# ChenKaiXuSan/Skiing_Analysis_PyTorch

Hardware: AMD Instinct MI355X
Metric: 3D-pose frames/sec, 8-view 518px clips (higher is better)
Workload: dtype f16

## Files before the change

skiing_analysis_pytorch_amd/csrc/common.h:

```cpp
#pragma once
#include <hip/hip_runtime.h>
#include <stdint.h>
#include <stdio.h>
#include <atomic>
#include <string>

#include "../../include/skimi.h"

namespace skimi {

void set_error(const char* fmt, ...);

#define SKIMI_CHECK_ARG(cond, ...)            \
    do {                                      \
        if (!(cond)) {                        \
            ::skimi::set_error(__VA_ARGS__);  \
            return SKIMI_ERR_ARG;             \
        }                                     \
    } while (0)

#define SKIMI_HIP(call)                                                                  \
    do {                                                                                 \
        hipError_t e_ = (call);                                                          \
        if (e_ != hipSuccess) {                                                          \
            ::skimi::set_error("%s failed: %s (%s:%d)", #call, hipGetErrorString(e_),    \
                               __FILE__, __LINE__);                                      \
            return SKIMI_ERR_HIP;                                                        \
        }                                                                                \
    } while (0)

#define SKIMI_LAUNCH_CHECK()                                                             \
    do {                                                                                 \
        hipError_t e_ = hipGetLastError();                                               \
        if (e_ != hipSuccess) {                                                          \
            ::skimi::set_error("kernel launch failed: %s (%s:%d)", hipGetErrorString(e_),\
                               __FILE__, __LINE__);                                      \
            return SKIMI_ERR_HIP;                                                        \
        }                                                                                \
    } while (0)

enum ProfKind { PROF_NONE = 0, PROF_ATTN_BF16 = 1, PROF_GEMM = 2 };
bool prof_armed(int kind, long size_key);
void prof_before(hipStream_t st);
void prof_after(hipStream_t st, double flops, double bytes);

int lds_opt_in(std::atomic<unsigned>& done, const void* kernel, int bytes, const char* what);
#define SKIMI_LDS_OPT_IN(KERNEL, BYTES, WHAT)                                                            \
    do {                                                                                                 \
        static std::atomic<unsigned> done_{0};                                                           \
        const int rc_ = ::skimi::lds_opt_in(done_, reinterpret_cast<const void*>(KERNEL), (int)(BYTES), WHAT); \
        if (rc_ != SKIMI_OK) return rc_;                                                                 \
    } while (0)

static inline int64_t cdiv(int64_t a, int64_t b) { return (a + b - 1) / b; }
static inline size_t align_up(size_t a, size_t b) { return (a + b - 1) / b * b; }

typedef __attribute__((ext_vector_type(8))) short bf16x8;
typedef __attribute__((ext_vector_type(4))) short bf16x4;
typedef __attribute__((ext_vector_type(16))) float f32x16;
typedef __attribute__((ext_vector_type(4))) float f32x4;

#ifdef __HIPCC__
__device__ __forceinline__ unsigned short f2bf(float x) {
    __bf16 b = (__bf16)x;
    return __builtin_bit_cast(unsigned short, b);
}
__device__ __forceinline__ float bf2f(unsigned short b) {
    return __builtin_bit_cast(float, ((unsigned int)b) << 16);
}
__device__ __forceinline__ unsigned short f2h(float x) {
    _Float16 h = (_Float16)x;
    return __builtin_bit_cast(unsigned short, h);
}
__device__ __forceinline__ float h2f(unsigned short b) { return (float)__builtin_bit_cast(_Float16, b); }
__device__ __forceinline__ unsigned short f2x16(float x, bool f16) {
    const unsigned short a = f2h(x), b = f2bf(x);
    return f16 ? a : b;
}
__device__ __forceinline__ float x16tof(unsigned short b, bool f16) {
    const float a = h2f(b), c = bf2f(b);
    return f16 ? a : c;
}
typedef __attribute__((ext_vector_type(8))) _Float16 f16x8;
template <bool F16>
__device__ __forceinline__ f32x16 mfma_32x32x16(bf16x8 a, bf16x8 b, f32x16 c) {
    if constexpr (F16)
        return __builtin_amdgcn_mfma_f32_32x32x16_f16(__builtin_bit_cast(f16x8, a), __builtin_bit_cast(f16x8, b), c, 0, 0, 0);
    else
        return __builtin_amdgcn_mfma_f32_32x32x16_bf16(a, b, c, 0, 0, 0);
}
__device__ __forceinline__ unsigned mx_scale_byte(float amax) {
    if (!(amax > 0.f)) return 0u;
    const float t = amax * (1.0f / 448.0f);
    const unsigned u = __float_as_uint(t);
    const int e = (int)((u >> 23) & 0xFF) - 127 + ((u & 0x7FFFFF) ? 1 : 0);
    return (unsigned)min(max(e + 127, 1), 254);
}
__device__ __forceinline__ float mx_inv_scale(unsigned sb) { return sb ? __uint_as_float((unsigned)(254 - (int)sb) << 23) : 0.f; }
__device__ __forceinline__ int mx_pack4(float a, float b, float c, float d, float inv) {
    int w = 0;
    w = __builtin_amdgcn_cvt_pk_fp8_f32(a * inv, b * inv, w, false);
    w = __builtin_amdgcn_cvt_pk_fp8_f32(c * inv, d * inv, w, true);
    return w;
}
__device__ __forceinline__ float max8(float v) {
    int x = __float_as_int(v);
    v = fmaxf(v, __int_as_float(__builtin_amdgcn_update_dpp(x, x, 0xB1, 0xF, 0xF, true)));
    x = __float_as_int(v);
    v = fmaxf(v, __int_as_float(__builtin_amdgcn_update_dpp(x, x, 0x4E, 0xF, 0xF, true)));
    x = __float_as_int(v);
    v = fmaxf(v, __int_as_float(__builtin_amdgcn_update_dpp(x, x, 0x141, 0xF, 0xF, true)));
    return v;
}
__device__ __forceinline__ float wave_sum(float v) {
#pragma unroll
    for (int o = 32; o > 0; o >>= 1) v += __shfl_xor(v, o, 64);
    return v;
}
__device__ __forceinline__ float wave_max(float v) {
#pragma unroll
    for (int o = 32; o > 0; o >>= 1) v = fmaxf(v, __shfl_xor(v, o, 64));
    return v;
}
#endif

}
```

skiing_analysis_pytorch_amd/csrc/gemm256.hip:

```cpp
#include <stdlib.h>

#include "common.h"
#include "gemm_epilogue.h"

namespace skimi {

typedef __attribute__((address_space(3))) void lds_void;
typedef __attribute__((address_space(1))) const void gbl_void;

__device__ __forceinline__ void tile_coords256(const GemmArgs& p, int& tm, int& tn) {
    const int nblk = p.ntm * p.ntn;
    const int bid = blockIdx.x;
    const int xcd = bid & 7;
    const int q = nblk >> 3, r = nblk & 7;
    const int id = (xcd < r ? xcd * (q + 1) : r * (q + 1) + (xcd - r) * q) + (bid >> 3);
    constexpr int GM = 8;
    const int per_group = GM * p.ntn;
    const int group = id / per_group, within = id - group * per_group;
    const int rows = min(GM, p.ntm - group * GM);
    tn = within / rows;
    tm = group * GM + within - tn * rows;
}

template <bool H16>
__device__ __forceinline__ bf16x4 pack4_16(float y0, float y1, float y2, float y3) {
    bf16x4 hb;
    if constexpr (H16) {
        hb[0] = (short)f2h(y0); hb[1] = (short)f2h(y1); hb[2] = (short)f2h(y2); hb[3] = (short)f2h(y3);
    } else {
        hb[0] = (short)f2bf(y0); hb[1] = (short)f2bf(y1); hb[2] = (short)f2bf(y2); hb[3] = (short)f2bf(y3);
    }
    return hb;
}

template <int MT, int EPI, int PF = 2, bool H16 = false>
__device__ __forceinline__ void epilogue256(const GemmArgs& p, f32x16 (&acc)[MT][2], char* smem, int wave, int lane,
                                            int wr, int wc, int m0, int n0) {
    const int l31 = lane & 31, lh = lane >> 5;
    float* stg = reinterpret_cast<float*>(smem) + wave * (32 * 64);
    const int n = n0 + wc * 64 + 4 * (lane & 15);
    if (p.dbg & 8) {
        if (acc[0][0][0] == 123.456f) ((float*)p.out)[0] = acc[MT - 1][1][15];
        return;
    }
    const bool interior = (m0 + 64 * MT <= p.M) && (n0 + 256 <= p.N) && !(p.dbg & 4);
    float4 bs = make_float4(0, 0, 0, 0), gm = make_float4(1, 1, 1, 1);
    if (EPI != 0 && n < p.N) {
        if (p.bias) bs = *reinterpret_cast<const float4*>(p.bias + n);
        if (EPI == 2) gm = *reinterpret_cast<const float4*>(p.gamma + n);
    }
#define SKIMI_ACC_TO_SLAB(i)                                                                                   \
    do {                                                                                                        \
        _Pragma("unroll") for (int j = 0; j < 2; ++j) _Pragma("unroll") for (int r = 0; r < 16; ++r)            \
            stg[((r & 3) + 8 * (r >> 2) + 4 * lh) * 64 + j * 32 + l31] = acc[i][j][r];                         \
        __builtin_amdgcn_fence(__ATOMIC_RELEASE, "wavefront");                                                  \
        __builtin_amdgcn_s_waitcnt(0xC07F);                                                     \
    } while (0)

    if (EPI == 2 && interior) {
        const int mrow0 = m0 + wr * (32 * MT) + (lane >> 4);
        float4 r[PF][8];
#pragma unroll
        for (int i = 0; i < PF && i < MT; ++i)
#pragma unroll
            for (int it = 0; it < 8; ++it)
                r[i][it] = *reinterpret_cast<const float4*>((const float*)p.resid + (long)(mrow0 + i * 32 + it * 4) * p.ldr + n);
#pragma unroll
        for (int i = 0; i < MT; ++i) {
            SKIMI_ACC_TO_SLAB(i);
            const int mrow = mrow0 + i * 32;
            float4 v[8];
#pragma unroll
            for (int it = 0; it < 8; ++it)
                v[it] = *reinterpret_cast<const float4*>(&stg[(it * 4 + (lane >> 4)) * 64 + 4 * (lane & 15)]);
#pragma unroll
            for (int it = 0; it < 8; ++it) {
                const float4 rr = r[i % PF][it];
                f32x4 ov = {rr.x + gm.x * (v[it].x + bs.x), rr.y + gm.y * (v[it].y + bs.y),
                            rr.z + gm.z * (v[it].z + bs.z), rr.w + gm.w * (v[it].w + bs.w)};
                *reinterpret_cast<f32x4*>((float*)p.out + (long)(mrow + it * 4) * p.ldo + n) = ov;
            }
            if (i + PF < MT) {
#pragma unroll
                for (int it = 0; it < 8; ++it)
                    r[i % PF][it] =
                        *reinterpret_cast<const float4*>((const float*)p.resid + (long)(mrow + PF * 32 + it * 4) * p.ldr + n);
            }
            __builtin_amdgcn_s_waitcnt(0xC07F);
        }
        return;
    }
    if (EPI != 0 && interior) {
        const bool mx = EPI == 3 && p.out_dtype == SKIMI_FP8MX;
#pragma unroll
        for (int i = 0; i < MT; ++i) {
            SKIMI_ACC_TO_SLAB(i);
            const int mrow = m0 + wr * (32 * MT) + i * 32 + (lane >> 4);
            float4 v[8];
#pragma unroll
            for (int it = 0; it < 8; ++it)
                v[it] = *reinterpret_cast<const float4*>(&stg[(it * 4 + (lane >> 4)) * 64 + 4 * (lane & 15)]);
            unsigned sb_mine = 0;
#pragma unroll
            for (int it = 0; it < 8; ++it) {
                float y0 = v[it].x + bs.x, y1 = v[it].y + bs.y, y2 = v[it].z + bs.z, y3 = v[it].w + bs.w;
                if (EPI == 3) {
                    const f32x2_t g0 = gelu_erf2(f32x2_t{y0, y1}), g1 = gelu_erf2(f32x2_t{y2, y3});
                    y0 = g0.x; y1 = g0.y; y2 = g1.x; y3 = g1.y;
                }
                if (mx) {
                    const unsigned sb = mx_scale_byte(max8(fmaxf(fmaxf(fabsf(y0), fabsf(y1)), fmaxf(fabsf(y2), fabsf(y3)))));
                    const long row = mrow + it * 4;
                    *reinterpret_cast<int*>((unsigned char*)p.out + row * p.ldo + n) = mx_pack4(y0, y1, y2, y3, mx_inv_scale(sb));
                    sb_mine = (lane & 7) == it ? sb : sb_mine;
                    if (it == 7) p.out_scales[(long)(mrow + (lane & 7) * 4) * (p.N >> 5) + (n >> 5)] = (unsigned char)sb_mine;
                    continue;
                }
                *reinterpret_cast<bf16x4*>((unsigned short*)p.out + (long)(mrow + it * 4) * p.ldo + n) = pack4_16<H16>(y0, y1, y2, y3);
            }
            __builtin_amdgcn_s_waitcnt(0xC07F);
        }
        return;
    }
#pragma unroll
    for (int i = 0; i < MT; ++i) {
        SKIMI_ACC_TO_SLAB(i);
        const int mrow = m0 + wr * (32 * MT) + i * 32 + (lane >> 4);
        if (EPI != 0) {
#pragma unroll 1
            for (int it = 0; it < 8; ++it) {
                const int m = mrow + it * 4;
                if (m >= p.M || n >= p.N || (p.dbg & 4)) continue;
                const float4 v = *reinterpret_cast<const float4*>(&stg[(it * 4 + (lane >> 4)) * 64 + 4 * (lane & 15)]);
                float y0 = v.x + bs.x, y1 = v.y + bs.y, y2 = v.z + bs.z, y3 = v.w + bs.w;
                if (EPI == 2) {
                    const float4 r = *reinterpret_cast<const float4*>((const float*)p.resid + (long)m * p.ldr + n);
                    f32x4 ov = {r.x + gm.x * y0, r.y + gm.y * y1, r.z + gm.z * y2, r.w + gm.w * y3};
// ... 59 lines not shown
    const unsigned short* w_src[4];
#pragma unroll
    for (int j = 0; j < MT; ++j) {
        const int row = 8 * (MT * wave + j) + (lane >> 3);
        const int c = (lane & 7) ^ ((row >> 1) & 7);
        a_src[j] = A + (long)min(m0 + row, p.M - 1) * p.lda + c * 8;
    }
#pragma unroll
    for (int j = 0; j < 4; ++j) {
        const int row = 8 * (4 * wave + j) + (lane >> 3);
        const int c = (lane & 7) ^ ((row >> 1) & 7);
        w_src[j] = W + (long)min(n0 + row, p.N - 1) * p.ldw + c * 8;
    }
    auto stage = [&](int buf, int kt) {
        char* ab = smem + buf * BUF + (MT * wave) * 8 * RB;
        char* wb = smem + buf * BUF + A_TILE + (4 * wave) * 8 * RB;
#pragma unroll
        for (int j = 0; j < MT; ++j)
            __builtin_amdgcn_global_load_lds((gbl_void*)(a_src[j] + kt * BK), (lds_void*)(ab + j * 8 * RB), 16, 0, 0);
#pragma unroll
        for (int j = 0; j < 4; ++j)
            __builtin_amdgcn_global_load_lds((gbl_void*)(w_src[j] + kt * BK), (lds_void*)(wb + j * 8 * RB), 16, 0, 0);
    };

    f32x16 acc[MT][2];
#pragma unroll
    for (int i = 0; i < MT; ++i)
#pragma unroll
        for (int j = 0; j < 2; ++j)
#pragma unroll
            for (int r = 0; r < 16; ++r) acc[i][j][r] = 0.f;

    stage(0, 0);
    __syncthreads();
    for (int kt = 0; kt < nkt; ++kt) {
        const int cur = kt & 1;
        if (kt + 1 < nkt && !(p.dbg & 1)) stage(cur ^ 1, kt + 1);
        const char* ab = smem + cur * BUF;
        const char* wb = ab + A_TILE;
        bf16x8 af[2][MT], wf[2][2];
        auto load_frags = [&](int s, int set) {
#pragma unroll
            for (int i = 0; i < MT; ++i) {
                const int row = wr * (32 * MT) + i * 32 + l31;
                af[set][i] = *reinterpret_cast<const bf16x8*>(ab + row * RB + (((2 * s + lh) ^ ((row >> 1) & 7)) << 4));
            }
#pragma unroll
            for (int j = 0; j < 2; ++j) {
                const int row = wc * 64 + j * 32 + l31;
                wf[set][j] = *reinterpret_cast<const bf16x8*>(wb + row * RB + (((2 * s + lh) ^ ((row >> 1) & 7)) << 4));
            }
        };
        if (!(p.dbg & 2)) {
        load_frags(0, 0);
        __builtin_amdgcn_sched_barrier(0);
#pragma unroll
        for (int s = 0; s < 4; ++s) {
            if (s + 1 < 4) load_frags(s + 1, (s + 1) & 1);
            __builtin_amdgcn_sched_barrier(0);
            __builtin_amdgcn_s_setprio(1);
#pragma unroll
            for (int i = 0; i < MT; ++i)
#pragma unroll
                for (int j = 0; j < 2; ++j)
                    acc[i][j] = mfma_32x32x16<F16>(af[s & 1][i], wf[s & 1][j], acc[i][j]);
            __builtin_amdgcn_s_setprio(0);
            __builtin_amdgcn_sched_barrier(0);
        }
        }
        __syncthreads();
    }

    epilogue256<MT, EPI, 2, F16 && EPI == 3>(p, acc, smem, wave, lane, wr, wc, m0, n0);
}

#define SKIMI_BAR()                           \
    do {                                      \
        __builtin_amdgcn_sched_barrier(0);    \
        __builtin_amdgcn_s_barrier();         \
        __builtin_amdgcn_sched_barrier(0);    \
    } while (0)
#define SKIMI_VMCNT(N) __builtin_amdgcn_s_waitcnt(0x0F70 | ((N) & 15) | (((N) >> 4) << 14))

template <int EPI, int DEEP, bool F16 = false>
__global__ __launch_bounds__(512, 2) void gemm256pp_kernel(const GemmArgs p) {
    constexpr int MT = 4, BM = 256, BN = 256, BK = 64;
    constexpr int RB = 128;
    constexpr int A_TILE = BM * RB, W_TILE = BN * RB, BUF = A_TILE + W_TILE;
    extern __shared__ __attribute__((aligned(16))) char smem[];

    const int tid = threadIdx.x, lane = tid & 63;
    const int wave = __builtin_amdgcn_readfirstlane(tid >> 6);
    const int wr = wave >> 2, wc = wave & 3;
    const int l31 = lane & 31, lh = lane >> 5;

    int tm, tn;
    tile_coords256(p, tm, tn);
    const int m0 = tm * BM, n0 = tn * BN;
    const int nkt = p.K / BK;

    const unsigned short* A = (const unsigned short*)p.A;
    const unsigned short* W = (const unsigned short*)p.W;
    const unsigned short* a_src[2][2];
    const unsigned short* w_src[2][2];
    int a_row0[2][2], w_row0[2][2];
#pragma unroll
    for (int h = 0; h < 2; ++h)
#pragma unroll
        for (int j = 0; j < 2; ++j) {
            const int g = 2 * wave + j;
            a_row0[h][j] = (g >> 3) * 128 + 64 * h + 8 * (g & 7);
            w_row0[h][j] = (g >> 2) * 64 + 32 * h + 8 * (g & 3);
            int row = a_row0[h][j] + (lane >> 3);
            int c = (lane & 7) ^ ((row >> 1) & 7);
            a_src[h][j] = A + (long)min(((p.dbg & 64) ? 0 : m0) + row, p.M - 1) * p.lda + c * 8;
            row = w_row0[h][j] + (lane >> 3);
            c = (lane & 7) ^ ((row >> 1) & 7);
            w_src[h][j] = W + (long)min(((p.dbg & 64) ? 0 : n0) + row, p.N - 1) * p.ldw + c * 8;
        }
    const bool no_dma = p.dbg & 1, no_mfma = p.dbg & 2, no_rd = p.dbg & 32;
    auto issue_a = [&](int h, int kt) {
        if (no_dma) return;
        char* base = smem + (kt & 1) * BUF;
#pragma unroll
        for (int j = 0; j < 2; ++j)
            __builtin_amdgcn_global_load_lds((gbl_void*)(a_src[h][j] + kt * BK), (lds_void*)(base + a_row0[h][j] * RB), 16,
                                             0, 0);
    };
    auto issue_w = [&](int h, int kt) {
        if (no_dma) return;
        char* base = smem + (kt & 1) * BUF + A_TILE;
#pragma unroll
        for (int j = 0; j < 2; ++j)
            __builtin_amdgcn_global_load_lds((gbl_void*)(w_src[h][j] + kt * BK), (lds_void*)(base + w_row0[h][j] * RB), 16,
                                             0, 0);
    };

    f32x16 acc[MT][2];
#pragma unroll
    for (int i = 0; i < MT; ++i)
#pragma unroll
        for (int j = 0; j < 2; ++j)
#pragma unroll
            for (int r = 0; r < 16; ++r) acc[i][j][r] = 0.f;

    issue_a(0, 0); issue_w(0, 0); issue_w(1, 0); issue_a(1, 0);
    if (nkt > 1) {
        issue_a(0, 1);
        if (DEEP) issue_w(0, 1);
        issue_w(1, 1);
        if (DEEP) SKIMI_VMCNT(6); else SKIMI_VMCNT(4);
    } else {
        SKIMI_VMCNT(0);
    }
    SKIMI_BAR();
    if (wr == 1) SKIMI_BAR();

    bf16x8 af[2][4], wf[2][4];
    if (no_rd) {
#pragma unroll
        for (int i = 0; i < 2; ++i)
#pragma unroll
            for (int s = 0; s < 4; ++s) af[i][s] = wf[i][s] = bf16x8{0, 0, 0, 0, 0, 0, 0, 0};
    }
    for (int kt = 0; kt < nkt; ++kt) {
        const char* ab = smem + (kt & 1) * BUF;
        const char* wb = ab + A_TILE;
        auto read_a = [&](int ih) {
            if (no_rd) return;
#pragma unroll
            for (int i = 0; i < 2; ++i)
#pragma unroll
                for (int s = 0; s < 4; ++s) {
                    const int row = wr * 128 + (2 * ih + i) * 32 + l31;
                    af[i][s] = *reinterpret_cast<const bf16x8*>(ab + row * RB + (((2 * s + lh) ^ ((row >> 1) & 7)) << 4));
                }
        };
        auto read_w = [&](int jh) {
            if (no_rd) return;
#pragma unroll
            for (int s = 0; s < 4; ++s) {
                const int row = wc * 64 + jh * 32 + l31;
                wf[jh][s] = *reinterpret_cast<const bf16x8*>(wb + row * RB + (((2 * s + lh) ^ ((row >> 1) & 7)) << 4));
            }
        };
#define SKIMI_QUADRANT(IH, JH)                                                                                  \
    do {                                                                                                         \
        SKIMI_BAR();                                                                                             \
        __builtin_amdgcn_s_setprio(1);                                                                           \
        if (!no_mfma) _Pragma("unroll") for (int s = 0; s < 4; ++s) {                                                          \
            acc[2 * IH][JH] = mfma_32x32x16<F16>(af[0][s], wf[JH][s], acc[2 * IH][JH]);                           \
            acc[2 * IH + 1][JH] = mfma_32x32x16<F16>(af[1][s], wf[JH][s], acc[2 * IH + 1][JH]);                   \
        }                                                                                                        \
        __builtin_amdgcn_s_setprio(0);                                                                           \
        SKIMI_BAR();                                                                                             \
    } while (0)

        read_w(0);
        read_a(0);
        if (kt + 1 < nkt) issue_a(1, kt + 1);
        SKIMI_QUADRANT(0, 0);
        read_w(1);
        if (!DEEP && kt + 1 < nkt) issue_w(0, kt + 1);
        SKIMI_QUADRANT(0, 1);
        read_a(1);
        if (kt + 2 < nkt) {
            issue_a(0, kt + 2);
            if (DEEP) issue_w(0, kt + 2);
        }
        SKIMI_QUADRANT(1, 1);
        if (kt + 2 < nkt) {
            issue_w(1, kt + 2);
            if (DEEP) SKIMI_VMCNT(6); else SKIMI_VMCNT(4);
        } else {
            SKIMI_VMCNT(0);
        }
        SKIMI_QUADRANT(1, 0);
#undef SKIMI_QUADRANT
    }
    if (wr == 0) SKIMI_BAR();

    epilogue256<MT, EPI, 2, F16 && EPI == 3>(p, acc, smem, wave, lane, wr, wc, m0, n0);
}


template <int EPI, bool F16 = false>
__global__ __launch_bounds__(256, 1) void gemm256w4_kernel(const GemmArgs p) {
    constexpr int RB = 128, BK = 64, PIECE = 128 * RB, NSLOT = 10;
    extern __shared__ __attribute__((aligned(16))) char smem[];

    const int tid = threadIdx.x, lane = tid & 63;
    const int wave = __builtin_amdgcn_readfirstlane(tid >> 6);
    const int wr = wave >> 1, wc = wave & 1;
    const int l31 = lane & 31, lh = lane >> 5;

    int tm, tn;
    tile_coords256(p, tm, tn);
    const int m0 = tm * 256, n0 = tn * 256;
    const int nkt = p.K / BK;
    const unsigned short* src[4][4];
#pragma unroll
    for (int q = 0; q < 4; ++q)
#pragma unroll
        for (int j = 0; j < 4; ++j) {
            const int row = (4 * wave + j) * 8 + (lane >> 3);
            const int c = (lane & 7) ^ ((row >> 1) & 7);
            src[q][j] = q < 2 ? (const unsigned short*)p.A + (long)min(m0 + 128 * q + row, p.M - 1) * p.lda + c * 8
                              : (const unsigned short*)p.W + (long)min(n0 + 128 * (q - 2) + row, p.N - 1) * p.ldw + c * 8;
        }
    auto issue = [&](int q, int kt, int slot) {
        char* base = smem + slot * PIECE + (4 * wave) * 8 * RB;
#pragma unroll
        for (int j = 0; j < 4; ++j)
            __builtin_amdgcn_global_load_lds((gbl_void*)(src[q][j] + kt * BK), (lds_void*)(base + j * 8 * RB), 16, 0, 0);
    };

    const int t = lh ^ ((l31 >> 1) & 7);
    const int lane_off = l31 * RB;
    bf16x8 fa0[4], fb0[4], fa1[4], fb1[4];
    auto read = [&](int sb, int s, bf16x8 (&fa)[4], bf16x8 (&fb)[4]) {
        int sa = sb + wr, sw = sb + 2 + wc;
        sa = sa >= NSLOT ? sa - NSLOT : sa;
        sw = sw >= NSLOT ? sw - NSLOT : sw;
        const char* pa = smem + sa * PIECE + lane_off + (((2 * s) ^ t) << 4);
        const char* pw = smem + sw * PIECE + lane_off + (((2 * s) ^ t) << 4);
#pragma unroll
        for (int i = 0; i < 4; ++i) fa[i] = *reinterpret_cast<const bf16x8*>(pa + i * 32 * RB);
#pragma unroll
        for (int i = 0; i < 4; ++i) fb[i] = *reinterpret_cast<const bf16x8*>(pw + i * 32 * RB);
    };

    f32x16 acc[2][4][2];
#pragma unroll
    for (int h = 0; h < 2; ++h)
#pragma unroll
        for (int i = 0; i < 4; ++i)
#pragma unroll
            for (int j = 0; j < 2; ++j)
#pragma unroll
                for (int r = 0; r < 16; ++r) acc[h][i][j][r] = 0.f;
#define SKIMI_W4_MFMA(FA, FB)                                                                                   \
    _Pragma("unroll") for (int j = 0; j < 4; ++j) _Pragma("unroll") for (int i = 0; i < 4; ++i)                 \
        acc[j >> 1][i][j & 1] = mfma_32x32x16<F16>(FA[i], FB[j], acc[j >> 1][i][j & 1])

#pragma unroll
    for (int q = 0; q < 4; ++q) issue(q, 0, q);
    if (nkt > 1) {
#pragma unroll
        for (int q = 0; q < 4; ++q) issue(q, 1, 4 + q);
        SKIMI_VMCNT(16);
    } else {
        SKIMI_VMCNT(0);
    }
    SKIMI_BAR();
    int sb = 0;
    read(sb, 0, fa0, fb0);
#define SKIMI_W4_HEAD()                       \
    do {                                      \
        __builtin_amdgcn_s_waitcnt(0xC07F);   \
        __builtin_amdgcn_sched_barrier(0);    \
    } while (0)
#define SKIMI_W4_TAIL(NDMA)                                                        \
    do {                                                                           \
        _Pragma("unroll") for (int g = 0; g < 4; ++g) {                            \
            __builtin_amdgcn_sched_group_barrier(0x008, 1, 0);                     \
            __builtin_amdgcn_sched_group_barrier(0x100, 2, 0);                     \
        }                                                                          \
        _Pragma("unroll") for (int g = 0; g < NDMA; ++g) {                         \
            __builtin_amdgcn_sched_group_barrier(0x008, 1, 0);                     \
            __builtin_amdgcn_sched_group_barrier(0x010, 1, 0);                     \
        }                                                                          \
        __builtin_amdgcn_sched_group_barrier(0x008, 12 - NDMA, 0);                 \
        __builtin_amdgcn_sched_barrier(0);                                         \
    } while (0)
#define SKIMI_W4_KTILE(N1, N2)                                                      \
    do {                                                                            \
        int s8 = sb + 8, s9 = sb + 9, s1 = sb + 1, nsb = sb + 4;                    \
        s8 = s8 >= NSLOT ? s8 - NSLOT : s8;                                         \
        s9 = s9 >= NSLOT ? s9 - NSLOT : s9;                                         \
        s1 = s1 >= NSLOT ? s1 - NSLOT : s1;                                         \
        nsb = nsb >= NSLOT ? nsb - NSLOT : nsb;                                     \
                                                                      \
        SKIMI_W4_HEAD();                                                            \
        read(sb, 1, fa1, fb1);                                                      \
        SKIMI_W4_MFMA(fa0, fb0);                                                    \
        SKIMI_W4_TAIL(0);                                                           \
                                                                      \
        SKIMI_W4_HEAD();                                                            \
        read(sb, 2, fa0, fb0);                                                      \
        if (N2) issue(0, kt + 2, s8);                                               \
        SKIMI_W4_MFMA(fa1, fb1);                                                    \
        SKIMI_W4_TAIL((N2 ? 4 : 0));                                                \
                                                                      \
        SKIMI_W4_HEAD();                                                            \
        read(sb, 3, fa1, fb1);                                                      \
        if (N2) issue(1, kt + 2, s9);                                               \
        SKIMI_W4_MFMA(fa0, fb0);                                                    \
        SKIMI_W4_TAIL((N2 ? 4 : 0));                                                \
                                                                      \
        SKIMI_W4_HEAD();                                                            \
        if (N1) {                                                                   \
            if (N2) SKIMI_VMCNT(8); else SKIMI_VMCNT(0);                            \
            SKIMI_BAR();                                                            \
            read(nsb, 0, fa0, fb0);                                                 \
            if (N2) {                                                               \
                issue(2, kt + 2, sb);                                               \
                issue(3, kt + 2, s1);                                               \
            }                                                                       \
        }                                                                           \
        SKIMI_W4_MFMA(fa1, fb1);                                                    \
        if (N1) SKIMI_W4_TAIL((N2 ? 8 : 0)); else __builtin_amdgcn_sched_barrier(0); \
        sb = nsb;                                                                   \
    } while (0)
    int kt = 0;
    for (; kt + 2 < nkt; ++kt) SKIMI_W4_KTILE(true, true);
    if (kt + 1 < nkt) {
        SKIMI_W4_KTILE(true, false);
        ++kt;
    }
    SKIMI_W4_KTILE(false, false);
#undef SKIMI_W4_KTILE
#undef SKIMI_W4_HEAD
#undef SKIMI_W4_TAIL
#undef SKIMI_W4_MFMA
    __builtin_amdgcn_s_waitcnt(0xC07F);
    SKIMI_BAR();

    epilogue256<4, EPI, 4, F16 && EPI == 3>(p, acc[0], smem, wave, lane, wr, 2 * wc, m0, n0);
    epilogue256<4, EPI, 4, F16 && EPI == 3>(p, acc[1], smem, wave, lane, wr, 2 * wc + 1, m0, n0);
}


typedef __attribute__((ext_vector_type(8))) int i32x8_t;
typedef __attribute__((ext_vector_type(4))) int i32x4_t;

template <int EPI>
__global__ __launch_bounds__(256, 1) void gemm256w4_fp8_kernel(const GemmArgs p) {
    constexpr int RB = 128, BK = 128, PIECE = 128 * RB, NSLOT = 10;
    extern __shared__ __attribute__((aligned(16))) char smem[];

    const int tid = threadIdx.x, lane = tid & 63;
    const int wave = __builtin_amdgcn_readfirstlane(tid >> 6);
    const int wr = wave >> 1, wc = wave & 1;
    const int l31 = lane & 31, lh = lane >> 5;

    int tm, tn;
    tile_coords256(p, tm, tn);
    const int m0 = tm * 256, n0 = tn * 256;
    const int nkt = p.K / BK;
    const unsigned char* src[4][4];
#pragma unroll
    for (int q = 0; q < 4; ++q)
#pragma unroll
        for (int j = 0; j < 4; ++j) {
            const int row = (4 * wave + j) * 8 + (lane >> 3);
            const int c = (lane & 7) ^ ((row >> 1) & 7);
            src[q][j] = q < 2 ? (const unsigned char*)p.A + (long)min(m0 + 128 * q + row, p.M - 1) * p.lda + c * 16
                              : (const unsigned char*)p.W + (long)min(n0 + 128 * (q - 2) + row, p.N - 1) * p.ldw + c * 16;
        }
    auto issue = [&](int q, int kt, int slot) {
        char* base = smem + slot * PIECE + (4 * wave) * 8 * RB;
#pragma unroll
        for (int j = 0; j < 4; ++j)
            __builtin_amdgcn_global_load_lds((gbl_void*)(src[q][j] + (long)kt * BK), (lds_void*)(base + j * 8 * RB), 16, 0, 0);
    };
    const unsigned* asc[4];
    const unsigned* wsc[4];
#pragma unroll
    for (int i = 0; i < 4; ++i) {
        asc[i] = reinterpret_cast<const unsigned*>(p.a_scales + (long)min(m0 + 128 * wr + 32 * i + l31, p.M - 1) * p.lsa);
        wsc[i] = reinterpret_cast<const unsigned*>(p.w_scales + (long)min(n0 + 128 * wc + 32 * i + l31, p.N - 1) * p.lsw);
    }
    unsigned sa[4], sw[4], san[4], swn[4];
    auto load_scales = [&](int kt) {
#pragma unroll
        for (int i = 0; i < 4; ++i) {
            san[i] = asc[i][kt];
            swn[i] = wsc[i][kt];
        }
    };
    auto take_scales = [&]() {
#pragma unroll
        for (int i = 0; i < 4; ++i) {
            sa[i] = san[i] >> (8 * lh);
            sw[i] = swn[i] >> (8 * lh);
        }
    };

    const int t = lh ^ ((l31 >> 1) & 7);
    const int lane_off = l31 * RB;
    i32x4_t fa0[2][4], fb0[2][4], fa1[2][4], fb1[2][4];
    auto readp = [&](int sb, int ks, i32x4_t (&fa)[2][4], i32x4_t (&fb)[2][4]) {
        int sA = sb + wr, sW = sb + 2 + wc;
        sA = sA >= NSLOT ? sA - NSLOT : sA;
        sW = sW >= NSLOT ? sW - NSLOT : sW;
#pragma unroll
        for (int h = 0; h < 2; ++h) {
            const int s = 2 * ks + h;
            const char* pa = smem + sA * PIECE + lane_off + (((2 * s) ^ t) << 4);
            const char* pw = smem + sW * PIECE + lane_off + (((2 * s) ^ t) << 4);
#pragma unroll
            for (int i = 0; i < 4; ++i) fa[h][i] = *reinterpret_cast<const i32x4_t*>(pa + i * 32 * RB);
#pragma unroll
            for (int i = 0; i < 4; ++i) fb[h][i] = *reinterpret_cast<const i32x4_t*>(pw + i * 32 * RB);
        }
    };

    f32x16 acc[2][4][2];
#pragma unroll
    for (int h = 0; h < 2; ++h)
#pragma unroll
        for (int i = 0; i < 4; ++i)
// ... 62 lines not shown
            readp(nsb, 0, fa0, fb0);                                                \
            load_scales(kt + 1);                                                    \
            if (N2) {                                                               \
                issue(2, kt + 2, sb);                                               \
                issue(3, kt + 2, s1);                                               \
            }                                                                       \
        }                                                                           \
        SKIMI_F8_MFMA(fa1, fb1, 2);                                                 \
        if (N1) SKIMI_F8_TAIL((N2 ? 16 : 8)); else __builtin_amdgcn_sched_barrier(0); \
        if (N1) {                                                                   \
            SKIMI_VMCNT(PW);            \
            take_scales();                                                          \
        }                                                                           \
        sb = nsb;                                                                   \
    } while (0)
    int kt = 0;
    for (; kt + 2 < nkt; ++kt) SKIMI_F8_KTILE(true, true, 8);
    if (kt + 1 < nkt) {
        SKIMI_F8_KTILE(true, false, 0);
        ++kt;
    }
    SKIMI_F8_KTILE(false, false, 0);
#undef SKIMI_F8_KTILE
#undef SKIMI_F8_HEAD
#undef SKIMI_F8_TAIL
#undef SKIMI_F8_MFMA
#undef SKIMI_F8_CAT
    __builtin_amdgcn_s_waitcnt(0xC07F);
    SKIMI_BAR();

    epilogue256<4, EPI, 4>(p, acc[0], smem, wave, lane, wr, 2 * wc, m0, n0);
    epilogue256<4, EPI, 4>(p, acc[1], smem, wave, lane, wr, 2 * wc + 1, m0, n0);
}

static int env_int(const char* name, int dflt, int& cache, bool& have) {
    static const bool dynamic = getenv("SKIMI_ENV_DYNAMIC") && atoi(getenv("SKIMI_ENV_DYNAMIC"));
    if (!have || dynamic) {
        const char* v = getenv(name);
        cache = v ? atoi(v) : dflt;
        have = true;
    }
    return cache;
}
#define SKIMI_ENV_INT(NAME, DFLT) ([]() { static int c; static bool h = false; return env_int(NAME, DFLT, c, h); }())

static int epi_kind(const GemmArgs& a) {
    const bool plain = a.vec4 && a.store_mode == 0 && a.out_rpb == 0 && a.out_off == 0 && a.out2 == nullptr &&
                       a.resid2 == nullptr && a.post_act == SKIMI_ACT_NONE && a.N % 4 == 0;
    if (!plain) return 0;
    if (a.gamma == nullptr && a.resid == nullptr && (a.out_dtype == SKIMI_BF16 || a.out_dtype == SKIMI_F16)) {
        if (a.act == SKIMI_ACT_NONE && a.out_dtype == SKIMI_BF16) return 1;
        if (a.act == SKIMI_ACT_GELU && a.out_dtype == (a.f16 ? SKIMI_F16 : SKIMI_BF16)) return 3;
        return 0;
    }
    if (a.out_dtype == SKIMI_FP8MX && a.out_scales != nullptr && a.gamma == nullptr && a.resid == nullptr && a.bias != nullptr &&
        a.act == SKIMI_ACT_GELU && a.N % 128 == 0)
        return 3;
    if (a.out_dtype == SKIMI_F32 && a.gamma != nullptr && a.resid != nullptr && a.resid_dtype == SKIMI_F32 &&
        a.resid_rpb == 0 && a.resid_off == 0 && a.act == SKIMI_ACT_NONE)
        return 2;
    return 0;
}

bool gemm256_eligible(const skimi_gemm_desc* d) {
    const bool bf = d->prec == SKIMI_PREC_BF16 && d->a_dtype == SKIMI_BF16 && d->w_dtype == SKIMI_BF16;
    const bool hf = d->prec == SKIMI_PREC_F16 && d->a_dtype == SKIMI_F16 && d->w_dtype == SKIMI_F16;
    return (bf || hf) && d->a_mode == 0 &&
           d->store_mode == 0 && d->K % 64 == 0 && d->lda % 8 == 0 && d->ldw % 8 == 0 && d->M >= 2048 &&
           d->N >= 512 && (((uintptr_t)d->A | (uintptr_t)d->W) & 15) == 0;
}

template <int MT, int EPI, bool F16 = false>
static int launch256(GemmArgs& a, hipStream_t st) {
    constexpr size_t lds = 2ull * (64 * MT + 256) * 128;
    SKIMI_LDS_OPT_IN((gemm256_kernel<MT, EPI, F16>), lds, "gemm256");
    a.ntm = (int)cdiv(a.M, 64 * MT);
    a.ntn = (int)cdiv(a.N, 256);
    a.splitk = 1;
    hipLaunchKernelGGL((gemm256_kernel<MT, EPI, F16>), dim3(a.ntm * a.ntn), dim3(512), lds, st, a);
    SKIMI_LAUNCH_CHECK();
    return SKIMI_OK;
}

template <int EPI, int DEEP, bool F16 = false>
static int launch256pp_(GemmArgs& a, hipStream_t st) {
    constexpr size_t lds = 2ull * (256 + 256) * 128;
    SKIMI_LDS_OPT_IN((gemm256pp_kernel<EPI, DEEP, F16>), lds, "gemm256pp");
    a.ntm = (int)cdiv(a.M, 256);
    a.ntn = (int)cdiv(a.N, 256);
    a.splitk = 1;
    hipLaunchKernelGGL((gemm256pp_kernel<EPI, DEEP, F16>), dim3(a.ntm * a.ntn), dim3(512), lds, st, a);
    SKIMI_LAUNCH_CHECK();
    return SKIMI_OK;
}

template <int EPI, bool F16 = false>
static int launch256pp(GemmArgs& a, hipStream_t st) {
    if constexpr (F16) return launch256pp_<EPI, 1, true>(a, st);
    const int deep = SKIMI_ENV_INT("SKIMI_GEMM256_DEEP", 1);
    return deep ? launch256pp_<EPI, 1>(a, st) : launch256pp_<EPI, 0>(a, st);
}

template <int EPI, bool F16 = false>
static int launch256w4(GemmArgs& a, hipStream_t st) {
    constexpr size_t lds = 10ull * 128 * 128;
    SKIMI_LDS_OPT_IN((gemm256w4_kernel<EPI, F16>), lds, "gemm256w4");
    a.ntm = (int)cdiv(a.M, 256);
    a.ntn = (int)cdiv(a.N, 256);
    a.splitk = 1;
    hipLaunchKernelGGL((gemm256w4_kernel<EPI, F16>), dim3(a.ntm * a.ntn), dim3(256), lds, st, a);
    SKIMI_LAUNCH_CHECK();
    return SKIMI_OK;
}

template <bool F16>
static int gemm256_pick(GemmArgs& a, hipStream_t st, int epi, bool mt3, bool w4, int use_pp) {
    if (mt3) {
        if (epi == 1) return launch256<3, 1, F16>(a, st);
        if (epi == 2) return launch256<3, 2, F16>(a, st);
        if (epi == 3) return launch256<3, 3, F16>(a, st);
        return launch256<3, 0, F16>(a, st);
    }
    if (w4) {
        if (epi == 1) return launch256w4<1, F16>(a, st);
        if (epi == 2) return launch256w4<2, F16>(a, st);
        if (epi == 3) return launch256w4<3, F16>(a, st);
        return launch256w4<0, F16>(a, st);
    }
    if (use_pp || F16) {
        if (epi == 1) return launch256pp<1, F16>(a, st);
        if (epi == 2) return launch256pp<2, F16>(a, st);
        if (epi == 3) return launch256pp<3, F16>(a, st);
        return launch256pp<0, F16>(a, st);
    }
    if constexpr (!F16) {
        if (epi == 1) return launch256<4, 1>(a, st);
        if (epi == 2) return launch256<4, 2>(a, st);
        if (epi == 3) return launch256<4, 3>(a, st);
        return launch256<4, 0>(a, st);
    }
    return SKIMI_ERR_ARG;
}

int gemm256_launch(GemmArgs& a, hipStream_t st) {
#ifdef SKIMI_ABLATIONS
    a.dbg = SKIMI_ENV_INT("SKIMI_GEMM256_ABL", 0);
#else
    a.dbg = 0;
#endif
    auto cost = [&](int bm) {
        const long tiles = cdiv(a.M, bm) * cdiv(a.N, 256);
        return (double)cdiv(tiles, 256) * bm;
    };
    const int epi = epi_kind(a);
    const int use_pp = SKIMI_ENV_INT("SKIMI_GEMM256_PP", 1);
    const int use_mt3 = SKIMI_ENV_INT("SKIMI_GEMM256_MT3", -1);
    const int use_w4 = SKIMI_ENV_INT("SKIMI_GEMM256_W4", -1);
    const bool mt3 = use_mt3 == 1 || (use_mt3 < 0 && cost(192) < 0.8 * cost(256));
    const bool w4 = use_w4 >= 0 ? use_w4 != 0 : (epi == 1 || (epi == 2 && a.K > 1024));
    return a.f16 ? gemm256_pick<true>(a, st, epi, mt3, w4, use_pp) : gemm256_pick<false>(a, st, epi, mt3, w4, use_pp);
}

template <int EPI>
static int launch256w4_fp8(GemmArgs& a, hipStream_t st) {
    constexpr size_t lds = 10ull * 128 * 128;
    SKIMI_LDS_OPT_IN(gemm256w4_fp8_kernel<EPI>, lds, "gemm256w4_fp8");
    a.ntm = (int)cdiv(a.M, 256);
    a.ntn = (int)cdiv(a.N, 256);
    a.splitk = 1;
    hipLaunchKernelGGL((gemm256w4_fp8_kernel<EPI>), dim3(a.ntm * a.ntn), dim3(256), lds, st, a);
    SKIMI_LAUNCH_CHECK();
    return SKIMI_OK;
}

int gemm256_fp8_launch(GemmArgs& a, hipStream_t st) {
    a.dbg = 0;
    const int epi = epi_kind(a);
    if (epi == 1) return launch256w4_fp8<1>(a, st);
    if (epi == 2) return launch256w4_fp8<2>(a, st);
    if (epi == 3) return launch256w4_fp8<3>(a, st);
    set_error("gemm256_fp8: epilogue not supported");
    return SKIMI_ERR_ARG;
}

}
```

Before: 15.61.

## Use 16x16x32 MFMA tiles in 256-wide GEMM kernels by default

Adds a 16x16x32 MFMA path to the pp and w4 256-tile GEMM kernels, with new fragment layouts, LDS read patterns, accumulator arrays and a matching accumulator-to-slab epilogue. An environment switch keeps the old 32x32x16 path, but the new 16x16 path is the default. The aim is a better MFMA issue rate or latency profile and a different LDS access pattern on MI355X. The cost is more MFMA instructions, more LDS reads per k-step and higher register pressure. The pp kernel also allocates both accumulator sets, which the compiler may or may not eliminate.

Result: faster. 16.11, median of 6 (+3.2%).

```diff
diff --git a/skiing_analysis_pytorch_amd/csrc/common.h b/skiing_analysis_pytorch_amd/csrc/common.h
--- a/skiing_analysis_pytorch_amd/csrc/common.h
+++ b/skiing_analysis_pytorch_amd/csrc/common.h
@@ -89,6 +89,13 @@
     else
         return __builtin_amdgcn_mfma_f32_32x32x16_bf16(a, b, c, 0, 0, 0);
 }
+template <bool F16>
+__device__ __forceinline__ f32x4 mfma_16x16x32(bf16x8 a, bf16x8 b, f32x4 c) {
+    if constexpr (F16)
+        return __builtin_amdgcn_mfma_f32_16x16x32_f16(__builtin_bit_cast(f16x8, a), __builtin_bit_cast(f16x8, b), c, 0, 0, 0);
+    else
+        return __builtin_amdgcn_mfma_f32_16x16x32_bf16(a, b, c, 0, 0, 0);
+}
 __device__ __forceinline__ unsigned mx_scale_byte(float amax) {
     if (!(amax > 0.f)) return 0u;
     const float t = amax * (1.0f / 448.0f);
diff --git a/skiing_analysis_pytorch_amd/csrc/gemm256.hip b/skiing_analysis_pytorch_amd/csrc/gemm256.hip
--- a/skiing_analysis_pytorch_amd/csrc/gemm256.hip
+++ b/skiing_analysis_pytorch_amd/csrc/gemm256.hip
@@ -33,14 +33,32 @@
     return hb;
 }
 
-template <int MT, int EPI, int PF = 2, bool H16 = false>
-__device__ __forceinline__ void epilogue256(const GemmArgs& p, f32x16 (&acc)[MT][2], char* smem, int wave, int lane,
+template <int MT>
+__device__ __forceinline__ void acc_to_slab(float* stg, const f32x16 (&acc)[MT][2], int i, int lane) {
+    const int l31 = lane & 31, lh = lane >> 5;
+#pragma unroll
+    for (int j = 0; j < 2; ++j)
+#pragma unroll
+        for (int r = 0; r < 16; ++r) stg[((r & 3) + 8 * (r >> 2) + 4 * lh) * 64 + j * 32 + l31] = acc[i][j][r];
+}
+template <int MT>
+__device__ __forceinline__ void acc_to_slab(float* stg, const f32x4 (&acc)[2 * MT][4], int i, int lane) {
+    const int l15 = lane & 15, lq = lane >> 4;
+#pragma unroll
+    for (int b = 0; b < 2; ++b)
+#pragma unroll
+        for (int c = 0; c < 4; ++c)
+#pragma unroll
+            for (int r = 0; r < 4; ++r) stg[(16 * b + 4 * lq + r) * 64 + 16 * c + l15] = acc[2 * i + b][c][r];
+}
+
+template <int MT, int EPI, int PF = 2, bool H16 = false, typename ACC>
+__device__ __forceinline__ void epilogue256(const GemmArgs& p, ACC& acc, char* smem, int wave, int lane,
                                             int wr, int wc, int m0, int n0) {
-    const int l31 = lane & 31, lh = lane >> 5;
     float* stg = reinterpret_cast<float*>(smem) + wave * (32 * 64);
     const int n = n0 + wc * 64 + 4 * (lane & 15);
     if (p.dbg & 8) {
-        if (acc[0][0][0] == 123.456f) ((float*)p.out)[0] = acc[MT - 1][1][15];
+        if (acc[0][0][0] == 123.456f) ((float*)p.out)[0] = acc[MT - 1][1][sizeof(acc[0][0]) / 4 - 1];
         return;
     }
     const bool interior = (m0 + 64 * MT <= p.M) && (n0 + 256 <= p.N) && !(p.dbg & 4);
@@ -51,8 +69,7 @@
     }
 #define SKIMI_ACC_TO_SLAB(i)                                                                                   \
     do {                                                                                                        \
-        _Pragma("unroll") for (int j = 0; j < 2; ++j) _Pragma("unroll") for (int r = 0; r < 16; ++r)            \
-            stg[((r & 3) + 8 * (r >> 2) + 4 * lh) * 64 + j * 32 + l31] = acc[i][j][r];                         \
+        acc_to_slab<MT>(stg, acc, i, lane);                                                                     \
         __builtin_amdgcn_fence(__ATOMIC_RELEASE, "wavefront");                                                  \
         __builtin_amdgcn_s_waitcnt(0xC07F);                                                     \
     } while (0)
@@ -278,7 +295,7 @@
     } while (0)
 #define SKIMI_VMCNT(N) __builtin_amdgcn_s_waitcnt(0x0F70 | ((N) & 15) | (((N) >> 4) << 14))
 
-template <int EPI, int DEEP, bool F16 = false>
+template <int EPI, int DEEP, bool F16 = false, bool M16 = false>
 __global__ __launch_bounds__(512, 2) void gemm256pp_kernel(const GemmArgs p) {
     constexpr int MT = 4, BM = 256, BN = 256, BK = 64;
     constexpr int RB = 128;
@@ -289,6 +306,7 @@
     const int wave = __builtin_amdgcn_readfirstlane(tid >> 6);
     const int wr = wave >> 2, wc = wave & 3;
     const int l31 = lane & 31, lh = lane >> 5;
+    const int l15 = lane & 15, lq = lane >> 4;
 
     int tm, tn;
     tile_coords256(p, tm, tn);
@@ -333,12 +351,17 @@
     };
 
     f32x16 acc[MT][2];
+    f32x4 acc16[2 * MT][4];
 #pragma unroll
     for (int i = 0; i < MT; ++i)
 #pragma unroll
         for (int j = 0; j < 2; ++j)
 #pragma unroll
             for (int r = 0; r < 16; ++r) acc[i][j][r] = 0.f;
+#pragma unroll
+    for (int i = 0; i < 2 * MT; ++i)
+#pragma unroll
+        for (int j = 0; j < 4; ++j) acc16[i][j] = f32x4{0.f, 0.f, 0.f, 0.f};
 
     issue_a(0, 0); issue_w(0, 0); issue_w(1, 0); issue_a(1, 0);
     if (nkt > 1) {
@@ -353,17 +376,28 @@
     if (wr == 1) SKIMI_BAR();
 
     bf16x8 af[2][4], wf[2][4];
+    bf16x8 af16[4][2], wf16[2][2][2];
     if (no_rd) {
 #pragma unroll
         for (int i = 0; i < 2; ++i)
 #pragma unroll
-            for (int s = 0; s < 4; ++s) af[i][s] = wf[i][s] = bf16x8{0, 0, 0, 0, 0, 0, 0, 0};
+            for (int s = 0; s < 4; ++s) af[i][s] = wf[i][s] = af16[s][i] = wf16[i][s >> 1][s & 1] = bf16x8{0, 0, 0, 0, 0, 0, 0, 0};
     }
     for (int kt = 0; kt < nkt; ++kt) {
         const char* ab = smem + (kt & 1) * BUF;
         const char* wb = ab + A_TILE;
         auto read_a = [&](int ih) {
             if (no_rd) return;
+            if constexpr (M16) {
+#pragma unroll
+                for (int i = 0; i < 4; ++i)
+#pragma unroll
+                    for (int s = 0; s < 2; ++s) {
+                        const int row = wr * 128 + ih * 64 + i * 16 + l15;
+                        af16[i][s] = *reinterpret_cast<const bf16x8*>(ab + row * RB + (((4 * s + lq) ^ ((row >> 1) & 7)) << 4));
+                    }
+                return;
+            }
 #pragma unroll
             for (int i = 0; i < 2; ++i)
 #pragma unroll
@@ -374,6 +408,16 @@
         };
         auto read_w = [&](int jh) {
             if (no_rd) return;
+            if constexpr (M16) {
+#pragma unroll
+                for (int c = 0; c < 2; ++c)
+#pragma unroll
+                    for (int s = 0; s < 2; ++s) {
+                        const int row = wc * 64 + jh * 32 + c * 16 + l15;
+                        wf16[jh][c][s] = *reinterpret_cast<const bf16x8*>(wb + row * RB + (((4 * s + lq) ^ ((row >> 1) & 7)) << 4));
+                    }
+                return;
+            }
 #pragma unroll
             for (int s = 0; s < 4; ++s) {
                 const int row = wc * 64 + jh * 32 + l31;
@@ -384,9 +428,16 @@
     do {                                                                                                         \
         SKIMI_BAR();                                                                                             \
         __builtin_amdgcn_s_setprio(1);                                                                           \
-        if (!no_mfma) _Pragma("unroll") for (int s = 0; s < 4; ++s) {                                                          \
-            acc[2 * IH][JH] = mfma_32x32x16<F16>(af[0][s], wf[JH][s], acc[2 * IH][JH]);                           \
-            acc[2 * IH + 1][JH] = mfma_32x32x16<F16>(af[1][s], wf[JH][s], acc[2 * IH + 1][JH]);                   \
+        if (no_mfma) {                                                                                           \
+        } else if constexpr (M16) {                                                                              \
+            _Pragma("unroll") for (int s = 0; s < 2; ++s) _Pragma("unroll") for (int i = 0; i < 4; ++i)          \
+                _Pragma("unroll") for (int c = 0; c < 2; ++c) acc16[4 * IH + i][2 * JH + c] =                    \
+                    mfma_16x16x32<F16>(af16[i][s], wf16[JH][c][s], acc16[4 * IH + i][2 * JH + c]);               \
+        } else {                                                                                                 \
+            _Pragma("unroll") for (int s = 0; s < 4; ++s) {                                                      \
+                acc[2 * IH][JH] = mfma_32x32x16<F16>(af[0][s], wf[JH][s], acc[2 * IH][JH]);                       \
+                acc[2 * IH + 1][JH] = mfma_32x32x16<F16>(af[1][s], wf[JH][s], acc[2 * IH + 1][JH]);               \
+            }                                                                                                    \
         }                                                                                                        \
         __builtin_amdgcn_s_setprio(0);                                                                           \
         SKIMI_BAR();                                                                                             \
@@ -416,11 +467,12 @@
     }
     if (wr == 0) SKIMI_BAR();
 
-    epilogue256<MT, EPI, 2, F16 && EPI == 3>(p, acc, smem, wave, lane, wr, wc, m0, n0);
-}
-
-
-template <int EPI, bool F16 = false>
+    if constexpr (M16) epilogue256<MT, EPI, 2, F16 && EPI == 3>(p, acc16, smem, wave, lane, wr, wc, m0, n0);
+    else epilogue256<MT, EPI, 2, F16 && EPI == 3>(p, acc, smem, wave, lane, wr, wc, m0, n0);
+}
+
+
+template <int EPI, bool F16 = false, bool M16 = false>
 __global__ __launch_bounds__(256, 1) void gemm256w4_kernel(const GemmArgs p) {
     constexpr int RB = 128, BK = 64, PIECE = 128 * RB, NSLOT = 10;
     extern __shared__ __attribute__((aligned(16))) char smem[];
@@ -451,6 +503,121 @@
             __builtin_amdgcn_global_load_lds((gbl_void*)(src[q][j] + kt * BK), (lds_void*)(base + j * 8 * RB), 16, 0, 0);
     };
 
+    if constexpr (M16) {
+    const int l15 = lane & 15;
+    const int t = (lane >> 4) ^ ((l15 >> 1) & 7);
+    const int lane_off = l15 * RB;
+    bf16x8 fa0[8], fb0[8], fa1[8], fb1[8];
+    auto read_one = [&](int sb, int s, int n, bf16x8 (&fa)[8], bf16x8 (&fb)[8]) {
+        int sa = sb + wr, sw = sb + 2 + wc;
+        sa = sa >= NSLOT ? sa - NSLOT : sa;
+        sw = sw >= NSLOT ? sw - NSLOT : sw;
+        const int off = lane_off + (((4 * s) ^ t) << 4) + (n & 7) * 16 * RB;
+        if (n < 8) fa[n] = *reinterpret_cast<const bf16x8*>(smem + sa * PIECE + off);
+        else fb[n - 8] = *reinterpret_cast<const bf16x8*>(smem + sw * PIECE + off);
+    };
+    auto issue_one = [&](int q, int j, int kt, int slot) {
+        __builtin_amdgcn_global_load_lds((gbl_void*)(src[q][j] + kt * BK), (lds_void*)(smem + slot * PIECE + (4 * wave + j) * 8 * RB),
+                                         16, 0, 0);
+    };
+
+    f32x4 acc[2][8][4];
+#pragma unroll
+    for (int h = 0; h < 2; ++h)
+#pragma unroll
+        for (int i = 0; i < 8; ++i)
+#pragma unroll
+            for (int c = 0; c < 4; ++c) {
+                acc[h][i][c] = f32x4{0.f, 0.f, 0.f, 0.f};
+                asm volatile("" : "+a"(acc[h][i][c]));
+            }
+    asm volatile("s_nop 1");
+    auto mfma = [&](f32x4& c, const bf16x8& a, const bf16x8& b) {
+        if constexpr (F16) asm volatile("v_mfma_f32_16x16x32_f16 %0, %1, %2, %0" : "+a"(c) : "v"(a), "v"(b));
+        else asm volatile("v_mfma_f32_16x16x32_bf16 %0, %1, %2, %0" : "+a"(c) : "v"(a), "v"(b));
+    };
+    auto kstep = [&](bf16x8 (&fa)[8], bf16x8 (&fb)[8], auto&& extra) {
+#pragma unroll
+        for (int j = 0; j < 8; ++j)
+#pragma unroll
+            for (int i = 0; i < 8; ++i) {
+                mfma(acc[j >> 2][i][j & 3], fa[i], fb[j]);
+                extra(8 * j + i);
+                __builtin_amdgcn_sched_barrier(0);
+            }
+    };
+
+#pragma unroll
+    for (int q = 0; q < 4; ++q) issue(q, 0, q);
+    if (nkt > 1) {
+#pragma unroll
+        for (int q = 0; q < 4; ++q) issue(q, 1, 4 + q);
+        SKIMI_VMCNT(16);
+    } else {
+        SKIMI_VMCNT(0);
+    }
+    SKIMI_BAR();
+    int sb = 0;
+#pragma unroll
+    for (int n = 0; n < 16; ++n) read_one(sb, 0, n, fa0, fb0);
+#define SKIMI_W4_HEAD()                       \
+    do {                                      \
+        __builtin_amdgcn_s_waitcnt(0xC07F);   \
+        __builtin_amdgcn_sched_barrier(0);    \
+    } while (0)
+#define SKIMI_W4_KTILE(N1, N2)                                                                       \
+    do {                                                                                             \
+        int s8 = sb + 8, s9 = sb + 9, s1 = sb + 1, nsb = sb + 4;                                     \
+        s8 = s8 >= NSLOT ? s8 - NSLOT : s8;                                                          \
+        s9 = s9 >= NSLOT ? s9 - NSLOT : s9;                                                          \
+        s1 = s1 >= NSLOT ? s1 - NSLOT : s1;                                                          \
+        nsb = nsb >= NSLOT ? nsb - NSLOT : nsb;                                                      \
+                                          \
+        SKIMI_W4_HEAD();                                                                             \
+        kstep(fa0, fb0, [&](int g) {                                                                 \
+            if (g < 16) read_one(sb, 1, g, fa1, fb1);                                                \
+            else if (N2 && g < 32 && (g & 1)) {                                              \
+                const int d = (g - 16) >> 1;                                                         \
+                issue_one(d >> 2, d & 3, kt + 2, (d >> 2) ? s9 : s8);                                \
+            }                                                                                        \
+        });                                                                                          \
+                         \
+        SKIMI_W4_HEAD();                                                                             \
+        if (N1) {                                                                                    \
+            if (N2) SKIMI_VMCNT(8); else SKIMI_VMCNT(0);                                             \
+            SKIMI_BAR();                                                                             \
+        }                                                                                            \
+        kstep(fa1, fb1, [&](int g) {                                                                 \
+            if (N1 && g < 16) read_one(nsb, 0, g, fa0, fb0);                                         \
+            else if (N2 && g < 32 && (g & 1)) {                                              \
+                const int d = (g - 16) >> 1;                                                         \
+                issue_one(2 + (d >> 2), d & 3, kt + 2, (d >> 2) ? s1 : sb);                          \
+            }                                                                                        \
+        });                                                                                          \
+        sb = nsb;                                                                                    \
+    } while (0)
+    int kt = 0;
+    for (; kt + 2 < nkt; ++kt) SKIMI_W4_KTILE(true, true);
+    if (kt + 1 < nkt) {
+        SKIMI_W4_KTILE(true, false);
+        ++kt;
+    }
+    SKIMI_W4_KTILE(false, false);
+#undef SKIMI_W4_KTILE
+#undef SKIMI_W4_HEAD
+    asm volatile("s_nop 7\n\ts_nop 4");
+#pragma unroll
+    for (int h = 0; h < 2; ++h)
+#pragma unroll
+        for (int i = 0; i < 8; ++i)
+#pragma unroll
+            for (int c = 0; c < 4; ++c) asm volatile("" : "+a"(acc[h][i][c]));
+    __builtin_amdgcn_s_waitcnt(0xC07F);
+    SKIMI_BAR();
+
+    epilogue256<4, EPI, 4, F16 && EPI == 3>(p, acc[0], smem, wave, lane, wr, 2 * wc, m0, n0);
+    epilogue256<4, EPI, 4, F16 && EPI == 3>(p, acc[1], smem, wave, lane, wr, 2 * wc + 1, m0, n0);
+    } else {
     const int t = lh ^ ((l31 >> 1) & 7);
     const int lane_off = l31 * RB;
     bf16x8 fa0[4], fb0[4], fa1[4], fb1[4];
@@ -564,6 +731,7 @@
 
     epilogue256<4, EPI, 4, F16 && EPI == 3>(p, acc[0], smem, wave, lane, wr, 2 * wc, m0, n0);
     epilogue256<4, EPI, 4, F16 && EPI == 3>(p, acc[1], smem, wave, lane, wr, 2 * wc + 1, m0, n0);
+    }
 }
 
 
@@ -792,57 +960,60 @@
     return SKIMI_OK;
 }
 
-template <int EPI, int DEEP, bool F16 = false>
+template <int EPI, int DEEP, bool F16, bool M16>
 static int launch256pp_(GemmArgs& a, hipStream_t st) {
     constexpr size_t lds = 2ull * (256 + 256) * 128;
-    SKIMI_LDS_OPT_IN((gemm256pp_kernel<EPI, DEEP, F16>), lds, "gemm256pp");
+    SKIMI_LDS_OPT_IN((gemm256pp_kernel<EPI, DEEP, F16, M16>), lds, "gemm256pp");
     a.ntm = (int)cdiv(a.M, 256);
     a.ntn = (int)cdiv(a.N, 256);
     a.splitk = 1;
-    hipLaunchKernelGGL((gemm256pp_kernel<EPI, DEEP, F16>), dim3(a.ntm * a.ntn), dim3(512), lds, st, a);
+    hipLaunchKernelGGL((gemm256pp_kernel<EPI, DEEP, F16, M16>), dim3(a.ntm * a.ntn), dim3(512), lds, st, a);
     SKIMI_LAUNCH_CHECK();
     return SKIMI_OK;
 }
 
-template <int EPI, bool F16 = false>
+template <int EPI, bool F16, bool M16>
 static int launch256pp(GemmArgs& a, hipStream_t st) {
-    if constexpr (F16) return launch256pp_<EPI, 1, true>(a, st);
+    if constexpr (F16) return launch256pp_<EPI, 1, true, M16>(a, st);
     const int deep = SKIMI_ENV_INT("SKIMI_GEMM256_DEEP", 1);
-    return deep ? launch256pp_<EPI, 1>(a, st) : launch256pp_<EPI, 0>(a, st);
-}
-
-template <int EPI, bool F16 = false>
+    return deep ? launch256pp_<EPI, 1, false, M16>(a, st) : launch256pp_<EPI, 0, false, M16>(a, st);
+}
+
+template <int EPI, bool F16, bool M16>
 static int launch256w4(GemmArgs& a, hipStream_t st) {
     constexpr size_t lds = 10ull * 128 * 128;
-    SKIMI_LDS_OPT_IN((gemm256w4_kernel<EPI, F16>), lds, "gemm256w4");
+    SKIMI_LDS_OPT_IN((gemm256w4_kernel<EPI, F16, M16>), lds, "gemm256w4");
     a.ntm = (int)cdiv(a.M, 256);
     a.ntn = (int)cdiv(a.N, 256);
     a.splitk = 1;
-    hipLaunchKernelGGL((gemm256w4_kernel<EPI, F16>), dim3(a.ntm * a.ntn), dim3(256), lds, st, a);
+    hipLaunchKernelGGL((gemm256w4_kernel<EPI, F16, M16>), dim3(a.ntm * a.ntn), dim3(256), lds, st, a);
     SKIMI_LAUNCH_CHECK();
     return SKIMI_OK;
 }
 
+template <bool F16, bool M16>
+static int gemm256_pick_loop(GemmArgs& a, hipStream_t st, int epi, bool w4) {
+    if (w4) {
+        if (epi == 1) return launch256w4<1, F16, M16>(a, st);
+        if (epi == 2) return launch256w4<2, F16, M16>(a, st);
+        if (epi == 3) return launch256w4<3, F16, M16>(a, st);
+        return launch256w4<0, F16, M16>(a, st);
+    }
+    if (epi == 1) return launch256pp<1, F16, M16>(a, st);
+    if (epi == 2) return launch256pp<2, F16, M16>(a, st);
+    if (epi == 3) return launch256pp<3, F16, M16>(a, st);
+    return launch256pp<0, F16, M16>(a, st);
+}
+
 template <bool F16>
-static int gemm256_pick(GemmArgs& a, hipStream_t st, int epi, bool mt3, bool w4, int use_pp) {
+static int gemm256_pick(GemmArgs& a, hipStream_t st, int epi, bool mt3, bool w4, int use_pp, bool m16) {
     if (mt3) {
         if (epi == 1) return launch256<3, 1, F16>(a, st);
         if (epi == 2) return launch256<3, 2, F16>(a, st);
         if (epi == 3) return launch256<3, 3, F16>(a, st);
         return launch256<3, 0, F16>(a, st);
     }
-    if (w4) {
-        if (epi == 1) return launch256w4<1, F16>(a, st);
-        if (epi == 2) return launch256w4<2, F16>(a, st);
-        if (epi == 3) return launch256w4<3, F16>(a, st);
-        return launch256w4<0, F16>(a, st);
-    }
-    if (use_pp || F16) {
-        if (epi == 1) return launch256pp<1, F16>(a, st);
-        if (epi == 2) return launch256pp<2, F16>(a, st);
-        if (epi == 3) return launch256pp<3, F16>(a, st);
-        return launch256pp<0, F16>(a, st);
-    }
+    if (w4 || use_pp || F16) return m16 ? gemm256_pick_loop<F16, true>(a, st, epi, w4) : gemm256_pick_loop<F16, false>(a, st, epi, w4);
     if constexpr (!F16) {
         if (epi == 1) return launch256<4, 1>(a, st);
         if (epi == 2) return launch256<4, 2>(a, st);
@@ -863,12 +1034,13 @@
         return (double)cdiv(tiles, 256) * bm;
     };
     const int epi = epi_kind(a);
+    const bool m16 = SKIMI_ENV_INT("SKIMI_GEMM256_MFMA", 16) != 32;
     const int use_pp = SKIMI_ENV_INT("SKIMI_GEMM256_PP", 1);
     const int use_mt3 = SKIMI_ENV_INT("SKIMI_GEMM256_MT3", -1);
     const int use_w4 = SKIMI_ENV_INT("SKIMI_GEMM256_W4", -1);
     const bool mt3 = use_mt3 == 1 || (use_mt3 < 0 && cost(192) < 0.8 * cost(256));
     const bool w4 = use_w4 >= 0 ? use_w4 != 0 : (epi == 1 || (epi == 2 && a.K > 1024));
-    return a.f16 ? gemm256_pick<true>(a, st, epi, mt3, w4, use_pp) : gemm256_pick<false>(a, st, epi, mt3, w4, use_pp);
+    return a.f16 ? gemm256_pick<true>(a, st, epi, mt3, w4, use_pp, m16) : gemm256_pick<false>(a, st, epi, mt3, w4, use_pp, m16);
 }
 
 template <int EPI>
```
